# AILab-CVC/CV-VAE

Measured on NVIDIA H100. Metric: video VAE encode+decode frames/sec at 17x576x1024, higher is better.
Workload: dtype fp16

## Files before the change

cvvae_b200/_lib.py:

```python
from __future__ import annotations

import ctypes as C
import os

from ._build import LIBPATH

F16, BF16, F32 = 0, 1, 2
PAD_ZERO, PAD_REPLICATE = 0, 1
CONV_BIAS_ALONG_M, CONV_FORCE_DIRECT, CONV_OUT_F32, CONV_W_PER_BATCH, CONV_X_SHARED = 1, 2, 4, 8, 16
ABI_VERSION = 3


class Tensor5(C.Structure):
    _fields_ = [
        ("ptr", C.c_void_p),
        ("B", C.c_int32), ("T", C.c_int32), ("H", C.c_int32), ("W", C.c_int32), ("C", C.c_int32),
        ("s_b", C.c_int64), ("s_t", C.c_int64), ("s_h", C.c_int64), ("s_w", C.c_int64), ("s_c", C.c_int64),
    ]


class ConvDesc(C.Structure):
    _fields_ = [
        ("x", Tensor5), ("y", Tensor5),
        ("w", C.c_void_p), ("w_ld", C.c_int64), ("bias", C.c_void_p), ("residual", C.c_void_p),
# ... 11 lines not shown

_P5 = C.POINTER(Tensor5)
_SIGNATURES = {
    "cvvae_conv3d": (C.c_int, [C.POINTER(ConvDesc), C.c_void_p]),
    "cvvae_conv3d_tc": (C.c_int, [C.POINTER(ConvDesc), C.c_void_p]),
    "cvvae_conv3d_direct": (C.c_int, [C.POINTER(ConvDesc), C.c_void_p]),
    "cvvae_conv3d_is_tc": (C.c_int, [C.POINTER(ConvDesc)]),
    "cvvae_conv3d_stacked": (C.c_int, [C.POINTER(ConvDesc), C.c_void_p]),
    "cvvae_pack_conv_weight": (C.c_int, [C.c_void_p, C.c_void_p, C.c_int32, C.c_int32, C.c_int32, C.c_int32, C.c_void_p]),
    "cvvae_groupnorm_stats": (C.c_int, [_P5, C.c_int32, C.c_int32, C.c_void_p, C.c_int32, C.c_void_p]),
    "cvvae_groupnorm_apply": (C.c_int, [_P5, _P5, C.c_int32, C.c_int32, C.c_void_p, C.c_void_p, C.c_void_p, C.c_float,
                                        C.c_int32, C.c_int32, C.c_void_p]),
    "cvvae_layernorm": (C.c_int, [_P5, _P5, C.c_void_p, C.c_void_p, C.c_float, C.c_int32, C.c_void_p]),
    "cvvae_softmax_rows": (C.c_int, [C.c_void_p, C.c_int64, C.c_void_p, C.c_int64, C.c_int64, C.c_int32, C.c_int32, C.c_void_p]),
    "cvvae_attn_temporal": (C.c_int, [_P5, _P5, _P5, _P5, C.c_int32, C.c_void_p]),
    "cvvae_replicate_border": (C.c_int, [_P5, C.c_int32, C.c_void_p]),
    "cvvae_copy5": (C.c_int, [_P5, _P5, C.c_int32, C.c_void_p]),
    "cvvae_pack_taps_hw": (C.c_int, [_P5, _P5, C.c_int32, C.c_int32, C.c_int32, C.c_int32, C.c_int32, C.c_int32, C.c_void_p]),
    "cvvae_blend": (C.c_int, [_P5, _P5, C.c_int32, C.c_int32, C.c_int32, C.c_void_p]),
    "cvvae_video_u8_to_f16": (C.c_int, [C.c_void_p, C.c_void_p, C.c_int32, C.c_int32, C.c_int32, C.c_int32, C.c_void_p]),
    "cvvae_video_f16_to_u8": (C.c_int, [C.c_void_p, C.c_void_p, C.c_int32, C.c_int32, C.c_int32, C.c_int32, C.c_void_p]),
    "cvvae_video_resize_u8": (C.c_int, [C.c_void_p, C.c_void_p, C.c_void_p, C.c_int32, C.c_int32, C.c_int32, C.c_int32, C.c_int32,
                                        C.c_int32, C.c_void_p]),
    "cvvae_conv_tc_set_trace": (C.c_int, [C.c_void_p, C.c_int32]),
    "cvvae_conv_tc_plan": (C.c_int, [C.POINTER(ConvDesc), C.POINTER(C.c_int32), C.c_int32]),
    "cvvae_last_error": (C.c_char_p, []),
    "cvvae_abi_version": (C.c_int, []),
    "cvvae_launch_count": (C.c_int64, []),
    "cvvae_probe_umma_shift": (C.c_int, [C.c_void_p, C.c_void_p, C.c_void_p, C.c_int32, C.c_int32, C.c_int32, C.c_int32, C.c_void_p]),
}
EXPORTS = tuple(_SIGNATURES)
CONV_TC_PLAN_FIELDS = ("eligible", "N_cta", "NACC", "TW", "ROWS", "TH", "tiles_w", "tiles_h", "n_tiles_n", "flat", "NA", "NB",
                       "grid", "vec2")

_lib = None


class CvvaeError(RuntimeError):
    pass


def load() -> C.CDLL:
    global _lib
    if _lib is not None:
        return _lib
    if not os.path.exists(LIBPATH):
        raise CvvaeError(
            f"{LIBPATH} is missing: build it with `python -c 'import __graft_entry__ as g; g.build()'` "
            "(cvvae_b200 has no CPU or PyTorch fallback path)")
    lib = C.CDLL(LIBPATH)
    for name, (res, args) in _SIGNATURES.items():
        fn = getattr(lib, name)
        fn.restype = res
        fn.argtypes = args
    if lib.cvvae_abi_version() != ABI_VERSION:
        raise CvvaeError(f"ABI mismatch: library {lib.cvvae_abi_version()} vs binding {ABI_VERSION}")
    _lib = lib
    return lib


def check(rc: int, what: str) -> None:
    if rc != 0:
        msg = load().cvvae_last_error().decode(errors="replace")
        raise CvvaeError(f"{what} failed ({rc}): {msg}")
```

cvvae_b200/csrc/conv_tc.cu:

```cuda
#include <stdlib.h>
#include <string.h>

#include "common.cuh"
#include "ptx.cuh"

namespace cvvae {

struct ConvTcParams {
  int B, T_in, T_out, H_out, W_out, Cin, Cout;
  int KT, KH, KW, st, sh, sw, off_t, off_h, off_w, pad_t;
  int up_time, flags;
  float alpha;
  int TW, ROWS, NACC, TH, N_cta, KHs, n_hgroups, slab_rows;
  int tiles_w, tiles_h, n_tiles_n, cblocks, flat;
  int NA, NB;
  uint32_t slab_bytes, slab_stride, b_bytes;
  const float* bias;
  const void* residual;
  void* y;
  long long ys_b, ys_t, ys_h, ys_w, ys_c;
  int yC, vec2;
  int64_t* gn_stats;
  int gn_groups, gn_cpg;
  int Cin2, cblocks2;
  unsigned long long* trace;
  int trace_n;
};

static constexpr int kThreads = 384;
static constexpr int kProducerRegs = 40, kMmaRegs = 232;
static constexpr uint32_t kBarBytes = 2048;

__device__ __forceinline__ void wait_bar(uint64_t* bar, uint32_t parity) { ptx::mbar_wait(bar, parity); }

struct TileCoord {
  int b, t, h0, w0, n0;
};

__device__ __forceinline__ TileCoord decode_tile(const ConvTcParams& p) {
  int id = static_cast<int>(blockIdx.x);
  TileCoord c;
  c.n0 = (id % p.n_tiles_n) * p.N_cta;
  id /= p.n_tiles_n;
  c.t = id % p.T_out;
  id /= p.T_out;
  c.w0 = (id % p.tiles_w) * (p.flat ? p.NACC * 128 : p.TW);
  id /= p.tiles_w;
  c.h0 = (id % p.tiles_h) * p.TH;
  c.b = id / p.tiles_h;
  return c;
}

template <class F>
__device__ __forceinline__ void for_each_slab(const ConvTcParams& p, int t, F&& f) {
  for (int kt = 0; kt < p.KT; ++kt) {
    int ti = t * p.st + kt + p.off_t;
    if (ti < 0 || ti >= p.T_in) {
      if (p.pad_t == CVVAE_PAD_ZERO) continue;
      ti = ti < 0 ? 0 : p.T_in - 1;
    }
    for (int hg = 0; hg < p.n_hgroups; ++hg)
      for (int kw = 0; kw < p.KW; ++kw)
        for (int cb = 0; cb < p.cblocks; ++cb) f(kt, ti, hg, kw, cb);
  }
}

template <int DT, int BN>
__global__ void __launch_bounds__(kThreads, 1)
    conv_tc_kernel(const __grid_constant__ CUtensorMap tmA, const __grid_constant__ CUtensorMap tmB,
                   const __grid_constant__ CUtensorMap tmA2, const __grid_constant__ CUtensorMap tmB2,
                   const ConvTcParams p) {
  constexpr int kMaxAcc = 256 / BN;
  constexpr int kR = BN / 2;
  using E = Elem<DT>;
  constexpr int kCB = 128 / static_cast<int>(sizeof(typename E::T));
  constexpr int kKmma = kCB / 4;
  constexpr int kKshift = kKmma == 16 ? 4 : 3;
  extern __shared__ uint8_t smem_raw[];
  uint8_t* smem = reinterpret_cast<uint8_t*>((reinterpret_cast<uintptr_t>(smem_raw) + 1023) & ~uintptr_t(1023));
  uint8_t* sA = smem;
  uint8_t* sB = sA + static_cast<size_t>(p.NA) * p.slab_stride;
  uint64_t* bars = reinterpret_cast<uint64_t*>(sB + static_cast<size_t>(p.NB) * p.b_bytes);
  uint64_t* fullA = bars;
  uint64_t* emptyA = bars + 8;
  uint64_t* fullB = bars + 16;
  uint64_t* emptyB = bars + 24;
  unsigned long long* gn_bins = reinterpret_cast<unsigned long long*>(bars + 64);

  const int warp = threadIdx.x >> 5;
  const int lane = threadIdx.x & 31;
  const bool traced = p.trace != nullptr && static_cast<int>(blockIdx.x) < p.trace_n;
  unsigned long long* trc = traced ? p.trace + static_cast<size_t>(blockIdx.x) * 8 : nullptr;
  if (traced && threadIdx.x == 0) trc[0] = ptx::globaltimer_ns();
  const TileCoord tc = decode_tile(p);
  int nacc_eff;
  if (p.flat) {
    nacc_eff = min(p.NACC, (p.W_out - tc.w0 + 127) / 128);
  } else {
    nacc_eff = max(0, min(p.NACC, (p.H_out - tc.h0 + p.ROWS - 1) / p.ROWS));
  }

  if (threadIdx.x < 128) gn_bins[threadIdx.x] = 0ull;
  if (threadIdx.x == 0) {
    for (int i = 0; i < p.NA; ++i) {
      ptx::mbar_init(&fullA[i], 1);
      ptx::mbar_init(&emptyA[i], 2);
    }
    for (int i = 0; i < p.NB; ++i) {
      ptx::mbar_init(&fullB[i], 1);
      ptx::mbar_init(&emptyB[i], 2);
    }
    ptx::fence_mbar_init();
    ptx::prefetch_tmap(&tmA);
    ptx::prefetch_tmap(&tmB);
  }
  __syncthreads();
  if (traced && threadIdx.x == 0) trc[1] = ptx::globaltimer_ns();

  if (threadIdx.x < 128) {
    ptx::setmaxnreg_dec<kProducerRegs>();
    int slot = 0;
    uint32_t phase = 0;
    auto advance = [&](int n) {
      __syncwarp();
      if (++slot == n) {
        slot = 0;
        phase ^= 1;
      }
    };
    if (warp == 0) {
      const int xb = (p.flags & CVVAE_CONV_X_SHARED) ? 0 : tc.b;
      for_each_slab(p, tc.t, [&](int kt, int ti, int hg, int kw, int cb) {
        wait_bar(&emptyA[slot], phase ^ 1);
        uint8_t* dst = sA + static_cast<size_t>(slot) * p.slab_stride;
        if (ptx::elect_one()) {
          if (p.flat) {
            ptx::mbar_expect_tx(&fullA[slot], static_cast<uint32_t>(nacc_eff) * 128u * 128u);
            for (int s = 0; s < nacc_eff; ++s)
              ptx::tma_load_5d(dst + s * 16384, &tmA, &fullA[slot], cb * kCB, tc.w0 + s * 128, 0, ti, xb);
          } else {
            ptx::mbar_expect_tx(&fullA[slot], p.slab_bytes);
            ptx::tma_load_5d(dst, &tmA, &fullA[slot], cb * kCB, tc.w0 * p.sw + kw + p.off_w,
                             tc.h0 * p.sh + hg * p.KHs + p.off_h, ti, xb);
          }
        }
        advance(p.NA);
      });
      for (int cb2 = 0; cb2 < p.cblocks2; ++cb2) {
        wait_bar(&emptyA[slot], phase ^ 1);
        if (ptx::elect_one()) {
          ptx::mbar_expect_tx(&fullA[slot], p.slab_bytes);
          ptx::tma_load_5d(sA + static_cast<size_t>(slot) * p.slab_stride, &tmA2, &fullA[slot], cb2 * kCB, tc.w0, tc.h0, tc.t, xb);
        }
        advance(p.NA);
      }
    } else if (warp == 1) {
      for_each_slab(p, tc.t, [&](int kt, int ti, int hg, int kw, int cb) {
        for (int khs = 0; khs < p.KHs; ++khs) {
          const int tap = (p.flags & CVVAE_CONV_W_PER_BATCH) ? tc.b : (kt * p.KH + hg * p.KHs + khs) * p.KW + kw;
          wait_bar(&emptyB[slot], phase ^ 1);
          if (ptx::elect_one()) {
            ptx::mbar_expect_tx(&fullB[slot], p.b_bytes);
            ptx::tma_load_3d(sB + static_cast<size_t>(slot) * p.b_bytes, &tmB, &fullB[slot], cb * kCB, tc.n0, tap);
          }
          advance(p.NB);
        }
      });
      for (int cb2 = 0; cb2 < p.cblocks2; ++cb2) {
        wait_bar(&emptyB[slot], phase ^ 1);
        if (ptx::elect_one()) {
          ptx::mbar_expect_tx(&fullB[slot], p.b_bytes);
          ptx::tma_load_3d(sB + static_cast<size_t>(slot) * p.b_bytes, &tmB2, &fullB[slot], cb2 * kCB, tc.n0, 0);
        }
        advance(p.NB);
      }
    }
    return;
  }

  ptx::setmaxnreg_inc<kMmaRegs>();
  const int half = (threadIdx.x >> 7) - 1;
  const bool wg_leader = (threadIdx.x & 127) == 0;
  float acc[kMaxAcc][kR];
  {
    int slotA = 0, slotB = 0;
    uint32_t phaseA = 0, phaseB = 0;
    int pendA = -1, pendB = -1;
    bool first = true;
    uint32_t accumulate = 0;
    const uint32_t sub_stride = p.flat ? 16384u : static_cast<uint32_t>(p.ROWS * p.TW) * 128u;
    const uint32_t tap_stride = static_cast<uint32_t>(p.TW) * 128u;
    const uint32_t half_off = static_cast<uint32_t>(half) * 8192u;
    auto mma_group = [&](uint32_t a_base, int ksteps, bool last_of_slab) {
      wait_bar(&fullB[slotB], phaseB);
      if (traced && first && threadIdx.x == 128) trc[3] = ptx::globaltimer_ns();
      first = false;
      const uint32_t b_base = ptx::smem_u32(sB + static_cast<size_t>(slotB) * p.b_bytes);
      if (nacc_eff == kMaxAcc && ksteps == 4) {
        ptx::wgmma_fence();
#pragma unroll
        for (int s = 0; s < kMaxAcc; ++s) {
          const uint32_t a_s = a_base + static_cast<uint32_t>(s) * sub_stride;
#pragma unroll
          for (int k = 0; k < 4; ++k)
            ptx::Wgmma<DT, BN>::run(acc[s], ptx::wgmma_desc_sw128(a_s + 32u * k), ptx::wgmma_desc_sw128(b_base + 32u * k),
                                    accumulate | static_cast<uint32_t>(k));
        }
        ptx::wgmma_commit();
      } else {
        ptx::wgmma_fence();
#pragma unroll
        for (int s = 0; s < kMaxAcc; ++s) {
          if (s < nacc_eff) {
            const uint32_t a_s = a_base + static_cast<uint32_t>(s) * sub_stride;
#pragma unroll
            for (int k = 0; k < 4; ++k)
// ... 17 lines not shown
        phaseB ^= 1;
      }
    };
    auto next_slab = [&]() {
      if (++slotA == p.NA) {
        slotA = 0;
        phaseA ^= 1;
      }
    };
    for_each_slab(p, tc.t, [&](int kt, int ti, int hg, int kw, int cb) {
      wait_bar(&fullA[slotA], phaseA);
      if (traced && slotA == 0 && phaseA == 0 && threadIdx.x == 128) trc[2] = ptx::globaltimer_ns();
      const int ch_left = p.Cin - cb * kCB;
      const int ksteps = ch_left >= kCB ? 4 : (ch_left + kKmma - 1) >> kKshift;
      const uint32_t a0 = ptx::smem_u32(sA + static_cast<size_t>(slotA) * p.slab_stride) + half_off;
      for (int khs = 0; khs < p.KHs; ++khs) mma_group(a0 + static_cast<uint32_t>(khs) * tap_stride, ksteps, khs == p.KHs - 1);
      next_slab();
    });
    for (int cb2 = 0; cb2 < p.cblocks2; ++cb2) {
      wait_bar(&fullA[slotA], phaseA);
      const int ch_left = p.Cin2 - cb2 * kCB;
      const int ksteps = ch_left >= kCB ? 4 : (ch_left + kKmma - 1) >> kKshift;
      mma_group(ptx::smem_u32(sA + static_cast<size_t>(slotA) * p.slab_stride) + half_off, ksteps, true);
      next_slab();
    }
    if (traced && threadIdx.x == 128) trc[4] = ptx::globaltimer_ns();
    ptx::wgmma_wait<0>();
#pragma unroll
    for (int s = 0; s < kMaxAcc; ++s) ptx::fence_regs(acc[s]);
    if (wg_leader) {
      if (pendB >= 0) ptx::mbar_arrive(&emptyB[pendB]);
      if (pendA >= 0) ptx::mbar_arrive(&emptyA[pendA]);
    }
  }
  if (traced && threadIdx.x == 128) trc[5] = ptx::globaltimer_ns();

  {
    using T = typename E::T;
    const int wl = warp & 3;
    const int cpair = 2 * (lane & 3);
    const int chalf = p.up_time == 2 ? p.Cout / 2 : p.Cout;
    const int bias_b = (p.flags & CVVAE_CONV_W_PER_BATCH) ? 0 : tc.b;
    const bool bias_m = p.bias && (p.flags & CVVAE_CONV_BIAS_ALONG_M);
    const bool out_f32 = (p.flags & CVVAE_CONV_OUT_F32) != 0;
    long long roff[kMaxAcc][2];
    bool rok[kMaxAcc][2];
    float rbias[kMaxAcc][2];
#pragma unroll
    for (int s = 0; s < kMaxAcc; ++s) {
#pragma unroll
      for (int rr = 0; rr < 2; ++rr) {
        const int m = half * 64 + wl * 16 + (lane >> 2) + rr * 8;
        int h, w;
        if (p.flat) {
          h = 0;
          w = tc.w0 + s * 128 + m;
        } else {
          h = tc.h0 + s * p.ROWS + m / p.TW;
          w = tc.w0 + m % p.TW;
        }
        rok[s][rr] = s < nacc_eff && h < p.H_out && w < p.W_out;
        roff[s][rr] = tc.b * p.ys_b + h * p.ys_h + w * p.ys_w;
        rbias[s][rr] = 0.f;
        if (bias_m && rok[s][rr]) {
          const long long m_index =
              ((static_cast<long long>(bias_b) * p.T_out + tc.t) * p.H_out + h) * static_cast<long long>(p.W_out) + w;
// ... 1 lines not shown
        }
      }
    }
    auto gn_add = [&](float gs0, float gq0, float gs1, float gq1, int cc, bool tok, bool c1ok) {
#pragma unroll
      for (int o = 4; o < 32; o <<= 1) {
        gs0 += __shfl_xor_sync(0xffffffffu, gs0, o);
        gq0 += __shfl_xor_sync(0xffffffffu, gq0, o);
        gs1 += __shfl_xor_sync(0xffffffffu, gs1, o);
        gq1 += __shfl_xor_sync(0xffffffffu, gq1, o);
      }
      if (p.gn_cpg == 1) {
        if (lane < 4 && tok) {
          atomicAdd(&gn_bins[cc * 2], gn_fix(gs0, kGnSumScale));
          atomicAdd(&gn_bins[cc * 2 + 1], gn_fix(gq0, kGnSqScale));
          if (c1ok) {
            atomicAdd(&gn_bins[(cc + 1) * 2], gn_fix(gs1, kGnSumScale));
            atomicAdd(&gn_bins[(cc + 1) * 2 + 1], gn_fix(gq1, kGnSqScale));
          }
        }
      } else {
        float ts = gs0 + gs1, tq = gq0 + gq1;
        for (int o = 1; o < (p.gn_cpg >> 1) && o < 4; o <<= 1) {
          ts += __shfl_xor_sync(0xffffffffu, ts, o);
          tq += __shfl_xor_sync(0xffffffffu, tq, o);
        }
        const int lanes_per_group = min(p.gn_cpg >> 1, 4);
        if (lane < 4 && (lane % lanes_per_group) == 0 && tok) {
          atomicAdd(&gn_bins[(cc / p.gn_cpg) * 2], gn_fix(ts, kGnSumScale));
          atomicAdd(&gn_bins[(cc / p.gn_cpg) * 2 + 1], gn_fix(tq, kGnSqScale));
        }
      }
    };
    const bool interior = nacc_eff == kMaxAcc && tc.n0 + BN <= p.Cout && !out_f32 && p.vec2 && !bias_m &&
                          (p.flat ? tc.w0 + kMaxAcc * 128 <= p.W_out
                                  : tc.h0 + kMaxAcc * p.ROWS <= p.H_out && tc.w0 + p.TW <= p.W_out);
    if (interior) {
#pragma unroll
      for (int j = 0; j < BN / 8; ++j) {
        const int cg = tc.n0 + 8 * j + cpair;
        const int n_il = p.up_time == 2 ? cg / chalf : 0;
        const int cc = cg - n_il * chalf;
        const int t_o = p.up_time == 2 ? 2 * tc.t + n_il - 1 : tc.t;
        const bool tok = t_o >= 0;
        const long long coff = t_o * p.ys_t + cc * p.ys_c;
        const float b0 = p.bias ? __ldg(p.bias + cg) : 0.f, b1 = p.bias ? __ldg(p.bias + cg + 1) : 0.f;
        float gs0 = 0.f, gq0 = 0.f, gs1 = 0.f, gq1 = 0.f;
        if (tok) {
#pragma unroll
          for (int s = 0; s < kMaxAcc; ++s) {
#pragma unroll
            for (int rr = 0; rr < 2; ++rr) {
              float a0 = fmaf(acc[s][4 * j + 2 * rr], p.alpha, b0);
              float a1 = fmaf(acc[s][4 * j + 2 * rr + 1], p.alpha, b1);
              const long long off = roff[s][rr] + coff;
              if (p.residual) {
                const float2 rf = E::to_f2(__ldg(reinterpret_cast<const typename E::P*>(reinterpret_cast<const T*>(p.residual) + off)));
                a0 += rf.x;
                a1 += rf.y;
              }
              const typename E::P o = E::pack2(a0, a1);
              *reinterpret_cast<typename E::P*>(reinterpret_cast<T*>(p.y) + off) = o;
              const float2 of = E::to_f2(o);
              gs0 += of.x;
              gq0 = fmaf(of.x, of.x, gq0);
              gs1 += of.y;
              gq1 = fmaf(of.y, of.y, gq1);
            }
          }
        }
// ... 52 lines not shown
              if (rp) {
                a0 += E::to_f(rp[0]);
                if (c1ok) a1 += E::to_f(rp[p.ys_c]);
              }
              const T o0 = E::from_f(a0), o1 = E::from_f(a1);
              yp[0] = o0;
              if (c1ok) yp[p.ys_c] = o1;
              a0 = E::to_f(o0);
              a1 = E::to_f(o1);
            }
            gs0 += a0;
            gq0 = fmaf(a0, a0, gq0);
            if (c1ok) {
              gs1 += a1;
              gq1 = fmaf(a1, a1, gq1);
            }
          }
        }
        if (p.gn_stats) gn_add(gs0, gq0, gs1, gq1, cc, tok, c1ok);
      }
    }
  }

  if (traced && threadIdx.x == 128) trc[6] = ptx::globaltimer_ns();
  if (p.gn_stats) {
    ptx::named_bar_sync(1, 256);
    const int ct = static_cast<int>(threadIdx.x) - 128;
    if (ct < 2 * p.gn_groups) {
      const unsigned long long vsum = gn_bins[ct];
      if (vsum != 0ull)
        atomicAdd(reinterpret_cast<unsigned long long*>(p.gn_stats) + static_cast<size_t>(tc.b) * 2 * p.gn_groups + ct, vsum);
    }
  }
  if (traced && threadIdx.x == 128) {
    unsigned smid;
    asm volatile("mov.u32 %0, %%smid;" : "=r"(smid));
    trc[7] = (ptx::globaltimer_ns() & 0xFFFFFFFFFFFFull) | (static_cast<unsigned long long>(smid) << 48);
  }
}

struct TmapKey {
  const void* ptr;
  uint32_t rank, swizzle, esz;
  cuuint64_t dims[5], strides[4];
  cuuint32_t box[5], estr[5];
  bool operator==(const TmapKey& o) const { return memcmp(this, &o, sizeof(TmapKey)) == 0; }
};
struct TmapSlot {
  TmapKey key;
  CUtensorMap map;
  bool valid;
};
static constexpr int kTmapSlots = 1024;

static int elem_bytes(int dtype) { return dtype == CVVAE_F32 ? 4 : 2; }
static int chan_block(int dtype) { return 128 / elem_bytes(dtype); }

static bool encode_map(CUtensorMap* m, const void* ptr, int rank, const cuuint64_t* dims, const cuuint64_t* strides_b,
                       const cuuint32_t* box, const cuuint32_t* estr, int esz,
                       CUtensorMapSwizzle swizzle = CU_TENSOR_MAP_SWIZZLE_128B) {
  static thread_local TmapSlot* cache = nullptr;
  if (!cache) cache = static_cast<TmapSlot*>(calloc(kTmapSlots, sizeof(TmapSlot)));
  TmapKey key;
  memset(&key, 0, sizeof(key));
  key.ptr = ptr;
  key.rank = static_cast<uint32_t>(rank);
// ... 38 lines not shown
}

bool conv_tc_eligible(const cvvae_conv_desc* d, const char** why) {
  const cvvae_tensor5& x = d->x;
  auto fail = [&](const char* m) {
    if (why) *why = m;
    return false;
  };
  if (x.s_c != 1) return fail("input channel stride != 1");
  if (d->w_ld % 8 != 0 || (d->w_ld == 0 && x.C % 8 != 0)) return fail("weight row stride not a 16-byte multiple");
  if ((x.s_w % 8) || (x.s_h % 8) || (x.s_t % 8) || (x.s_b % 8)) return fail("input strides not 16-byte multiples");
  if (reinterpret_cast<uintptr_t>(x.ptr) % 16) return fail("input pointer not 16-byte aligned");
  if (reinterpret_cast<uintptr_t>(d->w) % 16) return fail("weight pointer not 16-byte aligned");
  if (d->pad_hw != CVVAE_PAD_ZERO) {
    const int lo_h = d->off_h, hi_h = (d->y.H - 1) * d->sh + d->KH - 1 + d->off_h;
    const int lo_w = d->off_w, hi_w = (d->y.W - 1) * d->sw + d->KW - 1 + d->off_w;
    if (lo_h < 0 || lo_w < 0 || hi_h >= x.H || hi_w >= x.W) return fail("replicate H/W padding needs a pre-padded input");
  }
  if (d->sh > 2 || d->sw > 2 || d->sh != d->sw) return fail("unsupported spatial stride");
  if (d->KH > 3 || d->KW > 3 || d->KT > 3) return fail("kernel extent > 3");
  if (d->up_time == 2 && (d->Cout % 2)) return fail("odd Cout with up_time");
  return true;
}

static unsigned long long* g_trace_buf = nullptr;
static int g_trace_n = 0;
void conv_tc_set_trace(unsigned long long* buf, int n) {
  g_trace_buf = buf;
  g_trace_n = n;
}

template <int DT, int BN>
static int launch_bn(const CUtensorMap& tmA, const CUtensorMap& tmB, const CUtensorMap& tmA2, const CUtensorMap& tmB2,
                     const ConvTcParams& p, unsigned grid, size_t smem, cudaStream_t stream) {
  static PerDeviceOnce attr_set;
  if (attr_set.need()) {
    CVVAE_CUDA(cudaFuncSetAttribute(conv_tc_kernel<DT, BN>, cudaFuncAttributeMaxDynamicSharedMemorySize, 232448));
    attr_set.mark();
  }
  conv_tc_kernel<DT, BN><<<grid, kThreads, smem, stream>>>(tmA, tmB, tmA2, tmB2, p);
  return CVVAE_OK;
}

static int conv_tc_plan(const cvvae_conv_desc* d, ConvTcParams& p, size_t& smem, long long& grid) {
  const char* why = nullptr;
  if (!conv_tc_eligible(d, &why)) {
    set_error("cvvae_conv3d_tc: not eligible: %s", why);
    return CVVAE_E_UNSUPPORTED;
  }
  const cvvae_tensor5& x = d->x;
  const cvvae_tensor5& y = d->y;
  p = ConvTcParams{};
  p.B = x.B;
  p.T_in = x.T;
  p.Cin = x.C;
  p.Cout = d->Cout;
  p.up_time = d->up_time == 2 ? 2 : 1;
  p.T_out = p.up_time == 2 ? (y.T + 1) / 2 : y.T;
  p.H_out = y.H;
  p.W_out = y.W;
  p.KT = d->KT; p.KH = d->KH; p.KW = d->KW;
  p.st = d->st; p.sh = d->sh; p.sw = d->sw;
  p.off_t = d->off_t; p.off_h = d->off_h; p.off_w = d->off_w;
  p.pad_t = d->pad_t;
  p.flags = d->flags;
  p.alpha = d->alpha;
  p.bias = d->bias;
  p.residual = d->residual;
  p.y = y.ptr;
  p.ys_b = y.s_b; p.ys_t = y.s_t; p.ys_h = y.s_h; p.ys_w = y.s_w; p.ys_c = y.s_c;
  p.yC = y.C;
  if (d->flags & CVVAE_CONV_X_SHARED) CVVAE_CHECK_ARG(x.B == 1, "conv: CVVAE_CONV_X_SHARED needs x.B == 1");
  else CVVAE_CHECK_ARG(y.B == x.B, "conv: batch mismatch");
  if (d->flags & CVVAE_CONV_W_PER_BATCH)
// ... 40 lines not shown
        const long long tiles_h = (p.H_out + th - 1) / th;
        const long long cost = tiles_w * subtiles_h * 128 * 16 + tiles_w * tiles_h * (th + p.KHs - 1) * tw * 3;
        if (best_cost < 0 || cost < best_cost) {
          best_cost = cost;
          best_tw = tw;
        }
      }
      p.TW = best_tw;
      p.ROWS = 128 / p.TW;
      p.TH = p.ROWS * p.NACC;
      p.slab_rows = p.TH + p.KHs - 1;
      p.tiles_w = (p.W_out + p.TW - 1) / p.TW;
      p.tiles_h = (p.H_out + p.TH - 1) / p.TH;
    }
    const long long ctas_per_sample = 1ll * p.n_tiles_n * p.T_out * p.tiles_w * p.tiles_h;
    if (p.NACC <= 1 || ctas_per_sample >= num_sms()) break;
    p.NACC /= 2;
  }
  p.slab_bytes = p.flat ? static_cast<uint32_t>(p.NACC) * 16384u : static_cast<uint32_t>(p.slab_rows * p.TW) * 128u;
  p.slab_stride = (p.slab_bytes + 1023u) & ~1023u;
  p.b_bytes = static_cast<uint32_t>(N_cta) * 128u;

  const size_t budget = 232448 - 1024 - kBarBytes;
  int NB = 4;
  while (NB > 2 && static_cast<size_t>(NB) * p.b_bytes + 2ull * p.slab_stride > budget) --NB;
  const size_t rest = budget - static_cast<size_t>(NB) * p.b_bytes;
  int NA = static_cast<int>(rest / p.slab_stride);
  if (NA > 4) NA = 4;
  CVVAE_CHECK_ARG(NA >= 2, "conv_tc: slab of %u bytes does not fit the shared-memory budget", p.slab_bytes);
  while (NB < 8 && static_cast<size_t>(NB + 1) * p.b_bytes + static_cast<size_t>(NA) * p.slab_stride <= budget) ++NB;
  p.NA = NA;
  p.NB = NB;
  smem = 1024 + static_cast<size_t>(NA) * p.slab_stride + static_cast<size_t>(NB) * p.b_bytes + kBarBytes;

  grid = 1ll * p.n_tiles_n * p.T_out * p.tiles_w * p.tiles_h * p.B;
  CVVAE_CHECK_ARG(grid > 0 && grid < (1ll << 31), "conv_tc: grid size %lld out of range", grid);
  return CVVAE_OK;
}

int conv_tc_launch(const cvvae_conv_desc* d, cudaStream_t stream) {
  ConvTcParams p;
  size_t smem = 0;
  long long grid = 0;
  const int prc = conv_tc_plan(d, p, smem, grid);
  if (prc != CVVAE_OK) return prc;
  const cvvae_tensor5& x = d->x;
  const cvvae_tensor5& y = d->y;
  const int N_cta = p.N_cta;
  const int esz = elem_bytes(d->dtype);
  const int cb = chan_block(d->dtype);
  p.trace = g_trace_buf;
  p.trace_n = g_trace_n;

  CUtensorMap tmA, tmB;
  {
    cuuint64_t dims[5] = {(cuuint64_t)x.C, (cuuint64_t)x.W, (cuuint64_t)x.H, (cuuint64_t)x.T, (cuuint64_t)x.B};
    cuuint64_t strides[4] = {(cuuint64_t)x.s_w * esz, (cuuint64_t)x.s_h * esz, (cuuint64_t)x.s_t * esz, (cuuint64_t)x.s_b * esz};
    for (int i = 0; i < 4; ++i)
      if (dims[i + 1] == 1 && (strides[i] == 0 || strides[i] % 16)) strides[i] = (cuuint64_t)x.C * esz;
    cuuint32_t box[5], estr[5] = {1, (cuuint32_t)d->sw, (cuuint32_t)d->sh, 1, 1};
    box[0] = (cuuint32_t)cb;
    if (p.flat) {
      box[1] = 128; box[2] = 1;
    } else {
      box[1] = (cuuint32_t)(p.TW * d->sw);
      box[2] = (cuuint32_t)(p.slab_rows * d->sh);
// ... 27 lines not shown
                    "conv: fused shortcut needs the centre tap inside the kernel window");
    p.Cin2 = x2.C;
    p.cblocks2 = (x2.C + cb - 1) / cb;
    {
      cuuint64_t dims[5] = {(cuuint64_t)x2.C, (cuuint64_t)x2.W, (cuuint64_t)x2.H, (cuuint64_t)x2.T, (cuuint64_t)x2.B};
      cuuint64_t strides[4] = {(cuuint64_t)x2.s_w * esz, (cuuint64_t)x2.s_h * esz, (cuuint64_t)x2.s_t * esz, (cuuint64_t)x2.s_b * esz};
      for (int i = 0; i < 4; ++i)
        if (dims[i + 1] == 1 && (strides[i] == 0 || strides[i] % 16)) strides[i] = (cuuint64_t)x2.C * esz;
      cuuint32_t box[5] = {(cuuint32_t)cb, (cuuint32_t)p.TW, (cuuint32_t)p.slab_rows, 1, 1}, estr[5] = {1, 1, 1, 1, 1};
      if (!encode_map(&tmA2, x2.ptr, 5, dims, strides, box, estr, esz)) return CVVAE_E_CUDA;
    }
    {
      cuuint64_t dims[3] = {(cuuint64_t)x2.C, (cuuint64_t)p.Cout, 1};
      cuuint64_t strides[2] = {(cuuint64_t)x2.C * esz, (cuuint64_t)x2.C * p.Cout * esz};
      cuuint32_t box[3] = {(cuuint32_t)cb, (cuuint32_t)N_cta, 1}, estr[3] = {1, 1, 1};
      if (!encode_map(&tmB2, d->w2, 3, dims, strides, box, estr, esz)) return CVVAE_E_CUDA;
    }
  }

  p.gn_stats = nullptr;
  if (d->gn_stats) {
    const int cpg = d->gn_groups > 0 ? y.C / d->gn_groups : 0;
    const bool ok = !(d->flags & CVVAE_CONV_OUT_F32) && d->gn_groups > 0 && d->gn_groups <= 64 && y.C % d->gn_groups == 0 &&
                    cpg >= 1 && (cpg & (cpg - 1)) == 0;
    if (!ok) {
      set_error("conv_tc: fused GroupNorm statistics unsupported for this output (C=%d groups=%d)", y.C, d->gn_groups);
      return CVVAE_E_UNSUPPORTED;
    }
    p.gn_stats = d->gn_stats;
    p.gn_groups = d->gn_groups;
    p.gn_cpg = cpg;
  }

  int rc = CVVAE_OK;
  CVVAE_DISPATCH_DTYPE(d->dtype, {
    if (N_cta == 256) rc = launch_bn<DT, 256>(tmA, tmB, tmA2, tmB2, p, static_cast<unsigned>(grid), smem, stream);
    else if (N_cta == 128) rc = launch_bn<DT, 128>(tmA, tmB, tmA2, tmB2, p, static_cast<unsigned>(grid), smem, stream);
    else rc = launch_bn<DT, 64>(tmA, tmB, tmA2, tmB2, p, static_cast<unsigned>(grid), smem, stream);
  });
  if (rc != CVVAE_OK) return rc;
  CVVAE_LAUNCH_CHECK();
  return CVVAE_OK;
}

static int conv_tc_plan_query(const cvvae_conv_desc* d, int32_t* out, int32_t n) {
  ConvTcParams p;
  size_t smem = 0;
  long long grid = 0;
  const int rc = conv_tc_plan(d, p, smem, grid);
  if (rc != CVVAE_OK && rc != CVVAE_E_UNSUPPORTED) return rc;
  const bool ok = rc == CVVAE_OK;
  const int32_t v[] = {ok ? 1 : 0,
                       ok ? p.N_cta : 0,
                       ok ? p.NACC : 0,
                       ok ? p.TW : 0,
                       ok ? p.ROWS : 0,
                       ok ? p.TH : 0,
                       ok ? p.tiles_w : 0,
                       ok ? p.tiles_h : 0,
                       ok ? p.n_tiles_n : 0,
                       ok ? p.flat : 0,
                       ok ? p.NA : 0,
                       ok ? p.NB : 0,
                       ok ? static_cast<int32_t>(grid) : 0,
                       ok ? p.vec2 : 0};
  constexpr int32_t kFields = static_cast<int32_t>(sizeof(v) / sizeof(v[0]));
  for (int32_t i = 0; i < n && i < kFields; ++i) out[i] = v[i];
  return kFields;
}

}

extern "C" int cvvae_conv_tc_set_trace(void* device_buf, int32_t n_ctas) {
  cvvae::conv_tc_set_trace(static_cast<unsigned long long*>(device_buf), device_buf ? n_ctas : 0);
  return CVVAE_OK;
}

extern "C" int cvvae_conv_tc_plan(const cvvae_conv_desc* d, int32_t* out, int32_t n) {
  CVVAE_CHECK_ARG(d && cvvae::tensor_ok(&d->x) && cvvae::tensor_ok(&d->y) && d->w && (out || n <= 0),
                  "cvvae_conv_tc_plan: null argument");
  return cvvae::conv_tc_plan_query(d, out, n);
}

extern "C" int cvvae_conv3d_tc(const cvvae_conv_desc* d, void* stream) {
  CVVAE_CHECK_ARG(d && cvvae::tensor_ok(&d->x) && cvvae::tensor_ok(&d->y) && d->w, "cvvae_conv3d_tc: null argument");
  return cvvae::conv_tc_launch(d, static_cast<cudaStream_t>(stream));
}
```

cvvae_b200/csrc/ptx.cuh:

```cuda
#pragma once
#include <cuda.h>
#include <cuda_runtime.h>
#include <stdint.h>
#include <stdio.h>

#include "../../include/cvvae_b200.h"

namespace ptx {

__device__ __forceinline__ uint32_t smem_u32(const void* p) {
  return static_cast<uint32_t>(__cvta_generic_to_shared(p));
}

__device__ __forceinline__ bool elect_one() {
  uint32_t pred = 0;
  asm volatile(
      "{\n\t.reg .pred p;\n\t"
      "elect.sync _|p, 0xffffffff;\n\t"
      "selp.u32 %0, 1, 0, p;\n\t}\n"
      : "=r"(pred));
  return pred != 0;
}

__device__ __forceinline__ void mbar_init(uint64_t* bar, uint32_t count) {
// ... 50 lines not shown
}
__device__ __forceinline__ void tma_load_3d(void* smem_dst, const CUtensorMap* m, uint64_t* bar, int c0, int c1,
                                            int c2) {
  asm volatile(
      "cp.async.bulk.tensor.3d.shared::cluster.global.mbarrier::complete_tx::bytes [%0], [%1, {%3, %4, %5}], "
      "[%2];\n" ::"r"(smem_u32(smem_dst)),
      "l"(reinterpret_cast<uint64_t>(m)), "r"(smem_u32(bar)), "r"(c0), "r"(c1), "r"(c2)
      : "memory");
}

__device__ __forceinline__ void tma_store_5d(const CUtensorMap* m, const void* smem_src, int c0, int c1, int c2, int c3,
                                             int c4) {
  asm volatile(
      "cp.async.bulk.tensor.5d.global.shared::cta.bulk_group [%0, {%2, %3, %4, %5, %6}], [%1];\n" ::"l"(
          reinterpret_cast<uint64_t>(m)),
      "r"(smem_u32(smem_src)), "r"(c0), "r"(c1), "r"(c2), "r"(c3), "r"(c4)
      : "memory");
}
__device__ __forceinline__ void bulk_commit() { asm volatile("cp.async.bulk.commit_group;\n" ::: "memory"); }
template <int N>
__device__ __forceinline__ void bulk_wait_read() {
  asm volatile("cp.async.bulk.wait_group.read %0;\n" ::"n"(N) : "memory");
}
template <int N>
__device__ __forceinline__ void bulk_wait() {
  asm volatile("cp.async.bulk.wait_group %0;\n" ::"n"(N) : "memory");
}
__device__ __forceinline__ void st_shared_v4(uint32_t addr, uint32_t a, uint32_t b, uint32_t c, uint32_t d) {
  asm volatile("st.shared.v4.b32 [%0], {%1, %2, %3, %4};\n" ::"r"(addr), "r"(a), "r"(b), "r"(c), "r"(d) : "memory");
}
__device__ __forceinline__ uint4 ld_shared_v4(uint32_t addr) {
  uint4 v;
  asm volatile("ld.shared.v4.b32 {%0, %1, %2, %3}, [%4];\n" : "=r"(v.x), "=r"(v.y), "=r"(v.z), "=r"(v.w) : "r"(addr) : "memory");
  return v;
}

__device__ __forceinline__ uint64_t wgmma_desc_sw128(uint32_t saddr, uint32_t sbo_bytes = 1024) {
  uint64_t d = 0;
  d |= static_cast<uint64_t>((saddr >> 4) & 0x3FFF);
  d |= static_cast<uint64_t>(1) << 16;
  d |= static_cast<uint64_t>((sbo_bytes >> 4) & 0x3FFF) << 32;
  d |= static_cast<uint64_t>(1) << 62;
  return d;
}

__device__ __forceinline__ void wgmma_fence() { asm volatile("wgmma.fence.sync.aligned;\n" ::: "memory"); }
__device__ __forceinline__ void wgmma_commit() { asm volatile("wgmma.commit_group.sync.aligned;\n" ::: "memory"); }
template <int N>
__device__ __forceinline__ void wgmma_wait() {
  asm volatile("wgmma.wait_group.sync.aligned %0;\n" ::"n"(N) : "memory");
}
template <int R>
__device__ __forceinline__ void fence_regs(float (&d)[R]) {
#pragma unroll
  for (int i = 0; i < R; ++i) asm volatile("" : "+f"(d[i])::"memory");
}

template <int R>
__device__ __forceinline__ void setmaxnreg_dec() {
  asm volatile("setmaxnreg.dec.sync.aligned.u32 %0;\n" ::"n"(R));
}
template <int R>
__device__ __forceinline__ void setmaxnreg_inc() {
  asm volatile("setmaxnreg.inc.sync.aligned.u32 %0;\n" ::"n"(R));
}
__device__ __forceinline__ void named_bar_sync(int id, int nthreads) {
// ... 263 lines not shown
```

cvvae_b200/ops.py:

```python
from __future__ import annotations

import ctypes as C
from typing import Optional, Sequence, Tuple

import torch

from . import _lib as L

_DT = {torch.float16: L.F16, torch.bfloat16: L.BF16, torch.float32: L.F32}


def dtype_code(dt: torch.dtype) -> int:
    try:
        return _DT[dt]
    except KeyError:
        raise L.CvvaeError(f"cvvae_b200 computes in float16, bfloat16 or float32 (TF32 tensor-core products), got {dt}")


def _t5(t: torch.Tensor) -> L.Tensor5:
    assert t.dim() == 5, t.shape
    s = t.stride()
    return L.Tensor5(t.data_ptr(), t.shape[0], t.shape[1], t.shape[2], t.shape[3], t.shape[4], s[0], s[1], s[2], s[3], s[4])


# ... 80 lines not shown
                            w_per_batch=w_per_batch, x_shared=x_shared, sc_x=sc_x, sc_w=sc_w)
        B, T, H, W, Ci = x.shape
        if x_shared:
            B = out.shape[0]
        kt, kh, kw = kernel
        Co = d.Cout
        fn = {None: self.lib.cvvae_conv3d, "tc": self.lib.cvvae_conv3d_tc, "direct": self.lib.cvvae_conv3d_direct}[force]
        if self.profile is None:
            L.check(fn(C.byref(d), _stream(x)), "cvvae_conv3d")
            return out
        path = "conv_tc" if (force == "tc" or (force is None and self.lib.cvvae_conv3d_is_tc(C.byref(d)))) else "conv_direct"
        t_conv = (out.shape[1] + 1) // 2 if up_time == 2 else out.shape[1]
        mn = 2 * B * t_conv * out.shape[2] * out.shape[3] * Co * Ci
        if k_alg is not None:
            mn, kt, kh, kw, ref_taps = 2 * B * t_conv * out.shape[2] * out.shape[3] * Co, k_alg, 1, 1, None
        self.profile["flops"][path] += mn * kt * kh * kw
        self.profile["ref_flops"][path] += mn * (ref_taps if ref_taps is not None else kt * kh * kw)
        if sc_w is not None:
            sc = 2 * B * t_conv * out.shape[2] * out.shape[3] * Co * sc_x.shape[4]
            self.profile["flops"][path] += sc
            self.profile["ref_flops"][path] += sc
            self.profile["bytes"][path] += sc_x.numel() * sc_x.element_size() + sc_w.numel() * sc_w.element_size()
        self.profile["bytes"][path] += (x.numel() * x.element_size() + w.numel() * w.element_size() +
                                        out.numel() * out.element_size() * (2 if residual is not None else 1))
        self.profile["launches"][path] += 1
        s_ev, e_ev = torch.cuda.Event(enable_timing=True), torch.cuda.Event(enable_timing=True)
        s_ev.record()
        L.check(fn(C.byref(d), _stream(x)), "cvvae_conv3d")
        e_ev.record()
        self.profile["events"][path].append((s_ev, e_ev))
        return out

    @_on_tensor_device
    def conv_tc_plan(self, x: torch.Tensor, w: torch.Tensor, bias: Optional[torch.Tensor], **kw) -> dict:
        d = self._conv_desc(x, w, bias, **kw)
        n = len(L.CONV_TC_PLAN_FIELDS)
        vals = (C.c_int32 * n)()
        rc = self.lib.cvvae_conv_tc_plan(C.byref(d), vals, n)
        if rc < 0:
            L.check(rc, "cvvae_conv_tc_plan")
        return dict(zip(L.CONV_TC_PLAN_FIELDS, list(vals)))

    @staticmethod
    def _conv_desc(x, w, bias, *, kernel=(1, 1, 1), stride=(1, 1, 1), offset=(0, 0, 0), pad_t=L.PAD_ZERO, pad_hw=L.PAD_ZERO,
                   up_time=1, residual=None, alpha=1.0, out=None, out_f32=False, bias_along_m=False, w_ld=0, cout=None,
                   gn_stats=None, gn_groups=32, w_per_batch=False, x_shared=False, sc_x=None, sc_w=None) -> L.ConvDesc:
        kt, kh, kw = kernel
        st, sh, sw = stride
        ot, oh, ow = offset
        Co = cout if cout is not None else w.shape[1]
        if out is None:
            raise ValueError("conv(): the caller provides `out` (the engine knows the reference's output extents)")
        assert w.shape[0] == (out.shape[0] if w_per_batch else kt * kh * kw), (w.shape, kernel)
        d = L.ConvDesc()
        d.x = _t5(x)
        d.y = _t5(out)
        d.w = w.data_ptr()
        d.w_ld = w_ld
        d.bias = _ptr(bias)
        d.residual = _ptr(residual)
        d.Cout = Co
        d.KT, d.KH, d.KW = kt, kh, kw
        d.st, d.sh, d.sw = st, sh, sw
        d.off_t, d.off_h, d.off_w = ot, oh, ow
        d.pad_t, d.pad_hw = pad_t, pad_hw
        d.up_time = up_time
        d.dtype = dtype_code(x.dtype)
        d.flags = ((L.CONV_BIAS_ALONG_M if bias_along_m else 0) | (L.CONV_OUT_F32 if out_f32 else 0) |
                   (L.CONV_W_PER_BATCH if w_per_batch else 0) | (L.CONV_X_SHARED if x_shared else 0))
        d.alpha = alpha
        if gn_stats is not None:
            assert gn_stats.dtype == torch.int64 and gn_stats.is_contiguous()
            d.gn_stats = gn_stats.data_ptr()
            d.gn_groups = gn_groups
# ... 116 lines not shown
```

Measured before the change: 29.27.

## Stage conv epilogue through shared memory and write output with TMA stores

Adds a TMA-based epilogue to the tensor-core conv kernel for 16-bit dtypes. The producer warp reuses the A-slab ring to TMA-load residual tiles. The consumer warpgroups apply bias, alpha and residual, optionally gather GroupNorm stats, write the packed results into swizzled shared memory, and issue 5D TMA stores. This aims to replace scattered per-thread global stores and residual loads with bulk async transfers. The cost is extra pipeline slots, more synchronisation and new swizzle-indexing logic. It is on by default and can be disabled with an environment variable.

```diff
diff --git a/cvvae_b200/_lib.py b/cvvae_b200/_lib.py
--- a/cvvae_b200/_lib.py
+++ b/cvvae_b200/_lib.py
@@ -67,6 +67,7 @@
 EXPORTS = tuple(_SIGNATURES)
 CONV_TC_PLAN_FIELDS = ("eligible", "N_cta", "NACC", "TW", "ROWS", "TH", "tiles_w", "tiles_h", "n_tiles_n", "flat", "NA", "NB",
                        "grid", "vec2")
+CONV_TC_PLAN_EPILOGUE_FIELDS = CONV_TC_PLAN_FIELDS + ("tma_epilogue",)
 
 _lib = None
 
diff --git a/cvvae_b200/csrc/conv_tc.cu b/cvvae_b200/csrc/conv_tc.cu
--- a/cvvae_b200/csrc/conv_tc.cu
+++ b/cvvae_b200/csrc/conv_tc.cu
@@ -1,5 +1,7 @@
 #include <stdlib.h>
 #include <string.h>
+
+#include <type_traits>
 
 #include "common.cuh"
 #include "ptx.cuh"
@@ -23,6 +25,7 @@
   int64_t* gn_stats;
   int gn_groups, gn_cpg;
   int Cin2, cblocks2;
+  int tma_epi;
   unsigned long long* trace;
   int trace_n;
 };
@@ -65,10 +68,32 @@
   }
 }
 
+__device__ __forceinline__ bool epi_block(const ConvTcParams& p, const TileCoord& tc, int c, int cb, int& c0, int& t_o) {
+  const int g = tc.n0 + c * cb;
+  if (g >= p.Cout) return false;
+  const int n_il = p.up_time == 2 ? g / (p.Cout / 2) : 0;
+  c0 = g - n_il * (p.Cout / 2);
+  t_o = p.up_time == 2 ? 2 * tc.t + n_il - 1 : tc.t;
+  return t_o >= 0;
+}
+__device__ __forceinline__ void epi_piece(const ConvTcParams& p, const TileCoord& tc, int s, int hf, int& w, int& h) {
+  if (p.flat) {
+    w = tc.w0 + s * 128 + 64 * hf;
+    h = 0;
+  } else if (p.ROWS == 1) {
+    w = tc.w0 + 64 * hf;
+    h = tc.h0 + s;
+  } else {
+    w = tc.w0;
+    h = tc.h0 + s * p.ROWS + hf * (p.ROWS / 2);
+  }
+}
+
 template <int DT, int BN>
 __global__ void __launch_bounds__(kThreads, 1)
     conv_tc_kernel(const __grid_constant__ CUtensorMap tmA, const __grid_constant__ CUtensorMap tmB,
                    const __grid_constant__ CUtensorMap tmA2, const __grid_constant__ CUtensorMap tmB2,
+                   const __grid_constant__ CUtensorMap tmY, const __grid_constant__ CUtensorMap tmR,
                    const ConvTcParams p) {
   constexpr int kMaxAcc = 256 / BN;
   constexpr int kR = BN / 2;
@@ -113,6 +138,10 @@
     ptx::fence_mbar_init();
     ptx::prefetch_tmap(&tmA);
     ptx::prefetch_tmap(&tmB);
+    if (p.tma_epi) {
+      ptx::prefetch_tmap(&tmY);
+      if (p.residual) ptx::prefetch_tmap(&tmR);
+    }
   }
   __syncthreads();
   if (traced && threadIdx.x == 0) trc[1] = ptx::globaltimer_ns();
@@ -154,6 +183,29 @@
         }
         advance(p.NA);
       }
+      if (kCB == 64 && p.tma_epi) {
+        for (int c = 0; c < BN / kCB; ++c) {
+          int c0, t_o;
+          if (epi_block(p, tc, c, kCB, c0, t_o)) {
+            wait_bar(&emptyA[slot], phase ^ 1);
+            if (ptx::elect_one()) {
+              uint8_t* dst = sA + static_cast<size_t>(slot) * p.slab_stride;
+              if (p.residual) {
+                ptx::mbar_expect_tx(&fullA[slot], static_cast<uint32_t>(nacc_eff) * 16384u);
+                for (int s = 0; s < nacc_eff; ++s)
+                  for (int hf = 0; hf < 2; ++hf) {
+                    int w, h;
+                    epi_piece(p, tc, s, hf, w, h);
+                    ptx::tma_load_5d(dst + s * 16384 + hf * 8192, &tmR, &fullA[slot], c0, w, h, t_o, tc.b);
+                  }
+              } else {
+                ptx::mbar_arrive(&fullA[slot]);
+              }
+            }
+          }
+          advance(p.NA);
+        }
+      }
     } else if (warp == 1) {
       for_each_slab(p, tc.t, [&](int kt, int ti, int hg, int kw, int cb) {
         for (int khs = 0; khs < p.KHs; ++khs) {
@@ -182,6 +234,8 @@
   const int half = (threadIdx.x >> 7) - 1;
   const bool wg_leader = (threadIdx.x & 127) == 0;
   float acc[kMaxAcc][kR];
+  int epi_slot;
+  uint32_t epi_phase;
   {
     int slotA = 0, slotB = 0;
     uint32_t phaseA = 0, phaseB = 0;
@@ -265,6 +319,8 @@
       if (pendB >= 0) ptx::mbar_arrive(&emptyB[pendB]);
       if (pendA >= 0) ptx::mbar_arrive(&emptyA[pendA]);
     }
+    epi_slot = slotA;
+    epi_phase = phaseA;
   }
   if (traced && threadIdx.x == 128) trc[5] = ptx::globaltimer_ns();
 
@@ -332,10 +388,95 @@
         }
       }
     };
+    const bool tma_epi = kCB == 64 && p.tma_epi;
     const bool interior = nacc_eff == kMaxAcc && tc.n0 + BN <= p.Cout && !out_f32 && p.vec2 && !bias_m &&
                           (p.flat ? tc.w0 + kMaxAcc * 128 <= p.W_out
                                   : tc.h0 + kMaxAcc * p.ROWS <= p.H_out && tc.w0 + p.TW <= p.W_out);
-    if (interior) {
+    if (tma_epi) {
+      if constexpr (kCB == 64) {
+        constexpr int kBlocks = BN / kCB;
+        const int sw = lane >> 2;
+        const uint32_t row_off = static_cast<uint32_t>(half * 64 + wl * 16 + sw) * 128u + 4u * (lane & 3);
+        float bl[kBlocks][2];
+#pragma unroll
+        for (int c = 0; c < kBlocks; ++c) {
+          const int ch = tc.n0 + c * kCB + 8 * sw + cpair;
+          bl[c][0] = p.bias && ch < p.Cout ? __ldg(p.bias + ch) : 0.f;
+          bl[c][1] = p.bias && ch + 1 < p.Cout ? __ldg(p.bias + ch + 1) : 0.f;
+        }
+        auto stage_blocks = [&](auto res_c, auto gn_c, auto full_c) {
+          constexpr bool kRes = decltype(res_c)::value, kGn = decltype(gn_c)::value, kFull = decltype(full_c)::value;
+#pragma unroll
+          for (int c = 0; c < kBlocks; ++c) {
+            int c0, t_o;
+            if (!epi_block(p, tc, c, kCB, c0, t_o)) continue;
+            const int slot = epi_slot + c < p.NA ? epi_slot + c : epi_slot + c - p.NA;
+            const uint32_t stage = ptx::smem_u32(sA + static_cast<size_t>(slot) * p.slab_stride) + row_off;
+            wait_bar(&fullA[slot], epi_slot + c < p.NA ? epi_phase : epi_phase ^ 1);
+#pragma unroll
+            for (int jj = 0; jj < 8; ++jj) {
+              const int j = 8 * c + jj;
+              const float b0 = __shfl_sync(0xffffffffu, bl[c][0], 4 * jj + (lane & 3));
+              const float b1 = __shfl_sync(0xffffffffu, bl[c][1], 4 * jj + (lane & 3));
+              const uint32_t chunk = stage + static_cast<uint32_t>((jj ^ sw) << 4);
+              float gs0 = 0.f, gq0 = 0.f, gs1 = 0.f, gq1 = 0.f;
+#pragma unroll
+              for (int s = 0; s < kMaxAcc; ++s) {
+                const bool sok = kFull || s < nacc_eff;
+#pragma unroll
+                for (int rr = 0; rr < 2; ++rr) {
+                  const uint32_t addr = chunk + static_cast<uint32_t>(s * 16384 + rr * 1024);
+                  float a0 = fmaf(acc[s][4 * j + 2 * rr], p.alpha, b0);
+                  float a1 = fmaf(acc[s][4 * j + 2 * rr + 1], p.alpha, b1);
+                  if (kRes && sok) {
+                    const float2 rf = E::to_f2(ptx::ld_shared_b32(addr));
+                    a0 += rf.x;
+                    a1 += rf.y;
+                  }
+                  const uint32_t o = E::pack2(a0, a1);
+                  if (sok) ptx::st_shared_b32(addr, o);
+                  if (kGn && rok[s][rr]) {
+                    const float2 of = E::to_f2(o);
+                    gs0 += of.x;
+                    gq0 = fmaf(of.x, of.x, gq0);
+                    gs1 += of.y;
+                    gq1 = fmaf(of.y, of.y, gq1);
+                  }
+                }
+              }
+              if (kGn) gn_add(gs0, gq0, gs1, gq1, c0 + 8 * jj + cpair, tc.n0 + 8 * j < p.Cout, true);
+            }
+          }
+        };
+        auto by_full = [&](auto res_c, auto gn_c) {
+          if (nacc_eff == kMaxAcc) stage_blocks(res_c, gn_c, std::true_type{});
+          else stage_blocks(res_c, gn_c, std::false_type{});
+        };
+        auto by_gn = [&](auto res_c) {
+          if (p.gn_stats) by_full(res_c, std::true_type{});
+          else by_full(res_c, std::false_type{});
+        };
+        if (p.residual) by_gn(std::true_type{});
+        else by_gn(std::false_type{});
+        ptx::fence_proxy_async();
+        if (half == 0) ptx::named_bar_sync(3, 128);
+        else ptx::named_bar_sync(4, 128);
+        if (wg_leader) {
+          for (int c = 0; c < kBlocks; ++c) {
+            int bc0, bt;
+            if (!epi_block(p, tc, c, kCB, bc0, bt)) continue;
+            const int slot = epi_slot + c < p.NA ? epi_slot + c : epi_slot + c - p.NA;
+            const uint8_t* src = sA + static_cast<size_t>(slot) * p.slab_stride + half * 8192;
+            for (int s = 0; s < nacc_eff; ++s) {
+              int w, h;
+              epi_piece(p, tc, s, half, w, h);
+              ptx::tma_store_5d(&tmY, src + s * 16384, bc0, w, h, bt, tc.b);
+            }
+          }
+          ptx::bulk_commit();
+        }
+      }
+    } else if (interior) {
 #pragma unroll
       for (int j = 0; j < BN / 8; ++j) {
         const int cg = tc.n0 + 8 * j + cpair;
@@ -454,6 +595,7 @@
         atomicAdd(reinterpret_cast<unsigned long long*>(p.gn_stats) + static_cast<size_t>(tc.b) * 2 * p.gn_groups + ct, vsum);
     }
   }
+  if (kCB == 64 && p.tma_epi && wg_leader) ptx::bulk_wait_read<0>();
   if (traced && threadIdx.x == 128) {
     unsigned smid;
     asm volatile("mov.u32 %0, %%smid;" : "=r"(smid));
@@ -558,14 +700,41 @@
 
 template <int DT, int BN>
 static int launch_bn(const CUtensorMap& tmA, const CUtensorMap& tmB, const CUtensorMap& tmA2, const CUtensorMap& tmB2,
-                     const ConvTcParams& p, unsigned grid, size_t smem, cudaStream_t stream) {
+                     const CUtensorMap& tmY, const CUtensorMap& tmR, const ConvTcParams& p, unsigned grid, size_t smem,
+                     cudaStream_t stream) {
   static PerDeviceOnce attr_set;
   if (attr_set.need()) {
     CVVAE_CUDA(cudaFuncSetAttribute(conv_tc_kernel<DT, BN>, cudaFuncAttributeMaxDynamicSharedMemorySize, 232448));
     attr_set.mark();
   }
-  conv_tc_kernel<DT, BN><<<grid, kThreads, smem, stream>>>(tmA, tmB, tmA2, tmB2, p);
+  conv_tc_kernel<DT, BN><<<grid, kThreads, smem, stream>>>(tmA, tmB, tmA2, tmB2, tmY, tmR, p);
   return CVVAE_OK;
+}
+
+static bool y_map_strides(const cvvae_tensor5& y, int esz, cuuint64_t* strides) {
+  const long long s[4] = {y.s_w, y.s_h, y.s_t, y.s_b};
+  const int n[4] = {y.W, y.H, y.T, y.B};
+  if (y.s_c != 1 || reinterpret_cast<uintptr_t>(y.ptr) % 16) return false;
+  for (int i = 0; i < 4; ++i) {
+    if (n[i] == 1) {
+      strides[i] = (static_cast<cuuint64_t>(y.C) * esz + 15) & ~cuuint64_t(15);
+    } else {
+      if (s[i] <= 0 || (s[i] * esz) % 16) return false;
+      strides[i] = static_cast<cuuint64_t>(s[i]) * esz;
+    }
+  }
+  return true;
+}
+
+static bool tma_epilogue_ok(const cvvae_conv_desc* d, const ConvTcParams& p) {
+  const char* env = getenv("CVVAE_TMA_EPILOGUE");
+  if (env && strcmp(env, "0") == 0) return false;
+  if (d->dtype == CVVAE_F32 || (d->flags & (CVVAE_CONV_OUT_F32 | CVVAE_CONV_BIAS_ALONG_M))) return false;
+  cuuint64_t strides[4];
+  if (!y_map_strides(d->y, 2, strides)) return false;
+  if (d->residual && reinterpret_cast<uintptr_t>(d->residual) % 16) return false;
+  if (p.Cout % 8 || (p.up_time == 2 && (p.Cout / 2) % 64)) return false;
+  return p.N_cta / 64 <= p.NA;
 }
 
 static int conv_tc_plan(const cvvae_conv_desc* d, ConvTcParams& p, size_t& smem, long long& grid) {
@@ -672,6 +841,7 @@
   p.NA = NA;
   p.NB = NB;
   smem = 1024 + static_cast<size_t>(NA) * p.slab_stride + static_cast<size_t>(NB) * p.b_bytes + kBarBytes;
+  p.tma_epi = tma_epilogue_ok(d, p) ? 1 : 0;
 
   grid = 1ll * p.n_tiles_n * p.T_out * p.tiles_w * p.tiles_h * p.B;
   CVVAE_CHECK_ARG(grid > 0 && grid < (1ll << 31), "conv_tc: grid size %lld out of range", grid);
@@ -765,11 +935,23 @@
     p.gn_cpg = cpg;
   }
 
+  CUtensorMap tmY = tmA, tmR = tmA;
+  if (p.tma_epi) {
+    cuuint64_t dims[5] = {(cuuint64_t)y.C, (cuuint64_t)y.W, (cuuint64_t)y.H, (cuuint64_t)y.T, (cuuint64_t)y.B};
+    cuuint64_t strides[4];
+    y_map_strides(y, esz, strides);
+    const bool rows = p.ROWS >= 2;
+    cuuint32_t box[5] = {(cuuint32_t)cb, (cuuint32_t)(rows ? p.TW : 64), (cuuint32_t)(rows ? p.ROWS / 2 : 1), 1, 1},
+               estr[5] = {1, 1, 1, 1, 1};
+    if (!encode_map(&tmY, y.ptr, 5, dims, strides, box, estr, esz)) return CVVAE_E_CUDA;
+    if (d->residual && !encode_map(&tmR, d->residual, 5, dims, strides, box, estr, esz)) return CVVAE_E_CUDA;
+  }
+
   int rc = CVVAE_OK;
   CVVAE_DISPATCH_DTYPE(d->dtype, {
-    if (N_cta == 256) rc = launch_bn<DT, 256>(tmA, tmB, tmA2, tmB2, p, static_cast<unsigned>(grid), smem, stream);
-    else if (N_cta == 128) rc = launch_bn<DT, 128>(tmA, tmB, tmA2, tmB2, p, static_cast<unsigned>(grid), smem, stream);
-    else rc = launch_bn<DT, 64>(tmA, tmB, tmA2, tmB2, p, static_cast<unsigned>(grid), smem, stream);
+    if (N_cta == 256) rc = launch_bn<DT, 256>(tmA, tmB, tmA2, tmB2, tmY, tmR, p, static_cast<unsigned>(grid), smem, stream);
+    else if (N_cta == 128) rc = launch_bn<DT, 128>(tmA, tmB, tmA2, tmB2, tmY, tmR, p, static_cast<unsigned>(grid), smem, stream);
+    else rc = launch_bn<DT, 64>(tmA, tmB, tmA2, tmB2, tmY, tmR, p, static_cast<unsigned>(grid), smem, stream);
   });
   if (rc != CVVAE_OK) return rc;
   CVVAE_LAUNCH_CHECK();
@@ -796,7 +978,8 @@
                        ok ? p.NA : 0,
                        ok ? p.NB : 0,
                        ok ? static_cast<int32_t>(grid) : 0,
-                       ok ? p.vec2 : 0};
+                       ok ? p.vec2 : 0,
+                       ok ? p.tma_epi : 0};
   constexpr int32_t kFields = static_cast<int32_t>(sizeof(v) / sizeof(v[0]));
   for (int32_t i = 0; i < n && i < kFields; ++i) out[i] = v[i];
   return kFields;
diff --git a/cvvae_b200/csrc/ptx.cuh b/cvvae_b200/csrc/ptx.cuh
--- a/cvvae_b200/csrc/ptx.cuh
+++ b/cvvae_b200/csrc/ptx.cuh
@@ -106,6 +106,14 @@
 __device__ __forceinline__ uint4 ld_shared_v4(uint32_t addr) {
   uint4 v;
   asm volatile("ld.shared.v4.b32 {%0, %1, %2, %3}, [%4];\n" : "=r"(v.x), "=r"(v.y), "=r"(v.z), "=r"(v.w) : "r"(addr) : "memory");
+  return v;
+}
+__device__ __forceinline__ void st_shared_b32(uint32_t addr, uint32_t v) {
+  asm volatile("st.shared.b32 [%0], %1;\n" ::"r"(addr), "r"(v));
+}
+__device__ __forceinline__ uint32_t ld_shared_b32(uint32_t addr) {
+  uint32_t v;
+  asm volatile("ld.shared.b32 %0, [%1];\n" : "=r"(v) : "r"(addr));
   return v;
 }
 
diff --git a/cvvae_b200/ops.py b/cvvae_b200/ops.py
--- a/cvvae_b200/ops.py
+++ b/cvvae_b200/ops.py
@@ -136,14 +136,16 @@
         return out
 
     @_on_tensor_device
-    def conv_tc_plan(self, x: torch.Tensor, w: torch.Tensor, bias: Optional[torch.Tensor], **kw) -> dict:
+    def conv_tc_plan(self, x: torch.Tensor, w: torch.Tensor, bias: Optional[torch.Tensor], *, epilogue: bool = False,
+                     **kw) -> dict:
         d = self._conv_desc(x, w, bias, **kw)
-        n = len(L.CONV_TC_PLAN_FIELDS)
+        fields = L.CONV_TC_PLAN_EPILOGUE_FIELDS if epilogue else L.CONV_TC_PLAN_FIELDS
+        n = len(fields)
         vals = (C.c_int32 * n)()
         rc = self.lib.cvvae_conv_tc_plan(C.byref(d), vals, n)
         if rc < 0:
             L.check(rc, "cvvae_conv_tc_plan")
-        return dict(zip(L.CONV_TC_PLAN_FIELDS, list(vals)))
+        return dict(zip(fields, list(vals)))
 
     @staticmethod
     def _conv_desc(x, w, bias, *, kernel=(1, 1, 1), stride=(1, 1, 1), offset=(0, 0, 0), pad_t=L.PAD_ZERO, pad_hw=L.PAD_ZERO,
```

After: 30.35, median of 6. 3.7% higher.
